# kevlar-dev/kevlar

Measured on AMD Instinct MI355X. Metric: reads/sec through count+novel (3 samples, k=31), higher is better.
Workload: dtype u64 hash / u8 counters

## Files before the change

### kevlar_amd/csrc/kv_skm.hip

```cpp
#include <algorithm>
#include <cmath>

#include "kv_binned.h"
#include "kv_novel_device.h"
#include "kv_skm_device.h"

struct SkmGeom {
    int k, m, w, wpow;
    int kw, nbw, recw, ncap;
    uint32_t C1, F2, fbits;
    uint32_t nwg1, nwg2, quota1;
    uint32_t cap1, cap2;
    uint32_t np_max;
    uint64_t stride;
    uint64_t *seg1; uint32_t *cnt1;
    uint64_t *seg2; uint32_t *cnt2;
    uint64_t *loose; uint64_t loose_cap;
    unsigned long long *ctr;
    uint32_t n_buckets, quota3;
    uint32_t sbw;
    uint64_t bucket_kmers;
    uint32_t force_loose;
    uint64_t *abl_keys; uint8_t *abl_cnts; uint32_t *abl_bstart, *abl_bcount; uint32_t abl_cap_wg;
    uint64_t *dl_keys, *dl_hash; uint32_t *dl_bstart, *dl_bcount; uint32_t dl_cap_wg;
// ... 1310 lines not shown
        while (longer) {
            const uint32_t src = (uint32_t)__ffsll((long long)longer) - 1u;
            longer &= longer - 1ull;
            const uint64_t b0 = skm_shfl64(bw[0], src), b1 = skm_shfl64(bw[1], src), b2 = skm_shfl64(bw[2], src);
            const uint32_t nk_src = (uint32_t)__shfl((int)nk, (int)src);
            for (uint32_t j0 = 0; j0 < nk_src; j0 += 64) {
                const uint32_t j = j0 + lane;
                const bool live = j < nk_src;
                count_one(skm_kmer_at<KW>(b0, b1, b2, live ? j : 0u, k), live);
            }
        }
    }
    n_added = wave_sum_u64(n_added);
    if ((threadIdx.x & 63) == 0 && n_added) atomicAdd(&g.ctr[BIN_CTR_ADDED], (unsigned long long)n_added);
}

#define SKM_ROUTE_MAX_DEST 16
struct SkmOverflowSink { unsigned long long *ctr; uint64_t *ovf; uint8_t *ovf_dest; uint64_t ovf_cap; int ndest; };
__device__ __attribute__((noinline)) void skm_route_overflow(SkmOverflowSink rs, uint32_t d, uint64_t h, uint64_t count)
{
    {
        const unsigned long long here = __ballot(true);
        const uint32_t lane = threadIdx.x & 63u, leader = (uint32_t)__ffsll((long long)here) - 1u;
        unsigned long long o = 0;
        if (lane == leader) o = atomicAdd(&rs.ctr[ROUTE_CTR_OVERFLOW], (unsigned long long)__popcll(here));
        o = skm_shfl64(o, leader) + (unsigned long long)__popcll(here & ((1ull << lane) - 1ull));
        const bool fits = o < rs.ovf_cap;
        for (int dd = 0; dd < rs.ndest; ++dd) {
            const unsigned long long same = __ballot(fits && d == (uint32_t)dd);
            if (same && lane == (uint32_t)__ffsll((long long)same) - 1u) atomicAdd(&rs.ctr[ROUTE_CTR_DEST0 + dd], (unsigned long long)__popcll(same));
        }
        if (fits) {
            *(ulonglong2 *)(rs.ovf + 2 * o) = make_ulonglong2(h, count);
            rs.ovf_dest[o] = (uint8_t)d;
        }
    }
}

__device__ __forceinline__ void skm_route_item(const KvRouteSink &rs, const uint64_t *lo, uint32_t *cur, uint64_t h, uint64_t count)
{
    if (h == UINT64_MAX) return;
    uint32_t d = 0;
    for (int b = 1; b < rs.ndest; ++b) d += h >= lo[b] ? 1u : 0u;
    const uint32_t pos = cur ? atomicAdd(&cur[d], 1u) : 0xffffffffu;
    if (pos < rs.seg_cap) *(ulonglong2 *)(rs.seg + (((uint64_t)d * rs.nwg + blockIdx.x) * rs.seg_cap + pos) * 2) = make_ulonglong2(h, count);
    else skm_route_overflow(SkmOverflowSink{rs.ctr, rs.ovf, rs.ovf_dest, rs.ovf_cap, rs.ndest}, d, h, count);
}

template <int KW, int TS, bool COMPACT = false>
__global__ __launch_bounds__(SKM_THREADS3, 6) void k_skm_route(SkmGeom sg, HashParams hp, KvRouteSink rs)
{
    __shared__ SkmTable<KW, TS> tb;
    __shared__ uint32_t cnt[TS];
    __shared__ uint32_t next_bucket;
    __shared__ uint32_t cur[SKM_ROUTE_MAX_DEST];
    __shared__ uint64_t lo[SKM_ROUTE_MAX_DEST];
    __shared__ uint32_t dl_cur, dl_b0, dl_prev;
    __shared__ uint32_t dl_org, dl_lim;
    extern __shared__ __attribute__((aligned(16))) uint32_t dyn[];
    uint32_t *lut = dyn, *scratch = dyn + 256;
    if (threadIdx.x < 256) lut[threadIdx.x] = skm_ascii4(threadIdx.x);
    if (threadIdx.x < (uint32_t)rs.ndest) { cur[threadIdx.x] = 0; lo[threadIdx.x] = rs.bs * (uint64_t)threadIdx.x; }
    const int k = sg.k;
    uint64_t n_distinct = 0;
    skm_table_clear(tb);
    for (uint32_t i = threadIdx.x; i < TS; i += SKM_THREADS3) cnt[i] = 0;
    if (threadIdx.x == 0) {
        next_bucket = (uint32_t)atomicAdd(&sg.ctr[SKM_CTR_TICKET_COUNT], 1ull) * sg.bpt; dl_cur = 0; dl_b0 = 0; dl_prev = 0xffffffffu;
        dl_org = sg.dl_chunk ? 0u : blockIdx.x * sg.dl_cap_wg; dl_lim = sg.dl_chunk ? 0u : sg.dl_cap_wg;
    }
    auto dl_close = [&]() {
        if (sg.dl_keys && dl_prev != 0xffffffffu) {
            sg.dl_bstart[dl_prev] = dl_org + dl_b0;
            sg.dl_bcount[dl_prev] = dl_cur - dl_b0;
            if (sg.dl_chunk && dl_cur > dl_lim) atomicAdd(&sg.ctr[SKM_CTR_DL_RAN_OUT], 1ull);
        }
    };
    auto passes_of = [&](uint32_t b) {
        const uint32_t least = sg.passes > 1u ? sg.passes : 1u;
        const uint32_t *cnt2 = sg.cnt2 + (uint64_t)b * sg.nwg2;
        uint32_t nrec = 0;
        for (uint32_t s2 = 0; s2 < sg.nwg2; ++s2) nrec += cnt2[s2];
        const uint32_t per_pass = (uint32_t)TS * 13u / 20u;
        const uint32_t want = (19u * nrec / 10u + per_pass - 1u) / per_pass;
        return min(64u, max(least, want));
    };
    for (uint32_t taken = 0; taken < sg.quota3; ++taken) {
        __syncthreads();
        const uint32_t b = next_bucket;
        if (b >= sg.n_buckets) break;
        __syncthreads();
        if (threadIdx.x == 0) {
            dl_close();
            if (sg.dl_keys && sg.dl_chunk) {
                const uint32_t need = passes_of(b) * (uint32_t)TS;
                if (dl_cur + need > dl_lim) {
                    const unsigned long long c = atomicAdd(&sg.ctr[SKM_CTR_POOL_CHUNKS], 1ull);
                    if (c < sg.dl_nchunks && need <= sg.dl_chunk) { dl_org = (uint32_t)c * sg.dl_chunk; dl_lim = sg.dl_chunk; }
                    else { dl_org = 0; dl_lim = 0; atomicAdd(&sg.ctr[SKM_CTR_DL_RAN_OUT], 1ull); }
                    dl_cur = 0;
                }
            }
            dl_prev = b; dl_b0 = dl_cur;
            if ((b + 1u) & (sg.bpt - 1u)) next_bucket = b + 1u;
            else if (taken + 1 >= sg.quota3 || __hip_atomic_load(&sg.ctr[SKM_CTR_FAIL], __ATOMIC_RELAXED, __HIP_MEMORY_SCOPE_AGENT) != 0) next_bucket = 0xffffffffu;
            else next_bucket = (uint32_t)atomicAdd(&sg.ctr[SKM_CTR_TICKET_COUNT], 1ull) * sg.bpt;
        }
        const uint32_t passes = passes_of(b);
        for (uint32_t pass = 0; pass < passes; ++pass) {
        if (pass) __syncthreads();
        skm_walk_bucket<KW, false, 0, COMPACT>(sg, b, scratch, [&](const SkmKey<KW> &c, uint64_t) {
            if (!skm_cacheable<KW>(c)) return pass == 0u;
            if (passes > 1u && __umulhi(skm_slot_hash<KW>(c) * 0x9E3779B1u, passes) != pass) return false;
            const int slot = skm_table_insert(tb, c);
            if (slot >= 0) atomicAdd(&cnt[slot], 1u);
            return slot < 0;
        });
        __syncthreads();
        skm_for_occupied<TS>(tb.key[0], (uint16_t *)scratch, skm_wave_scratch_words(sg.sbw) * 2u, [&](uint32_t slot) {
            SkmKey<KW> c;
            c.w[0] = tb.key[0][slot];
            tb.key[0][slot] = SKM_EMPTY;
            if (KW == 2) { c.w[KW - 1] = tb.key[KW - 1][slot]; tb.key[KW - 1][slot] = SKM_EMPTY; }
            const uint32_t seen = cnt[slot];
            cnt[slot] = 0;
            n_distinct += 1;
            const uint64_t h = skm_key_hash<KW>(c, lut, hp);
            if (sg.dl_keys) {
                const unsigned long long here = __ballot(true);
                const uint32_t lane = threadIdx.x & 63u, leader = (uint32_t)__ffsll((long long)here) - 1u;
                uint32_t base = 0;
                if (lane == leader) base = atomicAdd(&dl_cur, (uint32_t)__popcll(here));
                base = (uint32_t)__shfl((int)base, (int)leader);
                const uint32_t at = base + (uint32_t)__popcll(here & ((1ull << lane) - 1ull));
                if (at < dl_lim) {
                    const uint64_t e = (uint64_t)dl_org + at;
                    sg.dl_keys[e * KW] = c.w[0];
                    if (KW == 2) sg.dl_keys[e * KW + (KW - 1)] = c.w[KW - 1];
                    sg.dl_hash[e] = h;
                }
            }
            skm_route_item(rs, lo, cur, h, seen);
        });
        }
    }
    __syncthreads();
    if (threadIdx.x == 0) {
        dl_close();
        if (sg.dl_keys && !sg.dl_chunk && dl_cur > sg.dl_cap_wg) atomicAdd(&sg.ctr[SKM_CTR_DL_RAN_OUT], 1ull);
    }
    if (threadIdx.x < (uint32_t)rs.ndest)
        rs.seg_count[(uint64_t)threadIdx.x * rs.nwg + blockIdx.x] = (uint32_t)min((uint64_t)cur[threadIdx.x], rs.seg_cap);
    n_distinct = wave_sum_u64(n_distinct);
    if ((threadIdx.x & 63) == 0 && n_distinct) atomicAdd(&sg.ctr[SKM_CTR_DISTINCT], (unsigned long long)n_distinct);
}

template <int KW>
__global__ __launch_bounds__(256) void k_skm_loose_route(SkmGeom sg, HashParams hp, KvRouteSink rs)
{
    __shared__ uint32_t lut[256];
    __shared__ uint64_t lo[SKM_ROUTE_MAX_DEST];
    __shared__ uint32_t dcount[SKM_ROUTE_MAX_DEST];
    __shared__ uint32_t wg_items, wg_cur;
    __shared__ unsigned long long wg_base;
    if (sg.ctr[SKM_CTR_FAIL] != 0) return;
    lut[threadIdx.x] = skm_ascii4(threadIdx.x);
    if (threadIdx.x < SKM_ROUTE_MAX_DEST) { lo[threadIdx.x] = rs.bs * (uint64_t)threadIdx.x; dcount[threadIdx.x] = 0; }
    if (threadIdx.x == 0) { wg_items = 0; wg_cur = 0; }
    __syncthreads();
    unsigned long long n = sg.ctr[SKM_CTR_LOOSE];
    if (n > sg.loose_cap) n = sg.loose_cap;
    const int k = sg.k, recw = sg.lrecw;
    {
        uint32_t mine = 0;
        for (uint64_t i = blockIdx.x * (uint64_t)blockDim.x + threadIdx.x; i < n; i += (uint64_t)gridDim.x * blockDim.x)
            mine += skm_hdr_n(sg.loose[i * (uint64_t)recw]);
        if (mine) atomicAdd(&wg_items, mine);
    }
    __syncthreads();
    if (threadIdx.x == 0) wg_base = wg_items ? atomicAdd(&rs.ctr[ROUTE_CTR_OVERFLOW], (unsigned long long)wg_items) : 0ull;
    __syncthreads();
    for (uint64_t i = blockIdx.x * (uint64_t)blockDim.x + threadIdx.x; i < n; i += (uint64_t)gridDim.x * blockDim.x) {
        const uint64_t *rec = sg.loose + i * (uint64_t)recw;
        uint64_t bw[3];
#pragma unroll
        for (int t = 0; t < 3; ++t) bw[t] = t < sg.nbw ? rec[1 + t] : 0ull;
        const uint32_t nk = skm_hdr_n(rec[0]);
        SkmKey<KW> fw = skm_first_kmer<KW>(bw, k);
        SkmKey<KW> rc = skm_revcomp<KW>(fw, k);
        for (uint32_t j = 0; j < nk; ++j) {
            if (j) skm_roll<KW>(fw, rc, skm_base_at(bw, j + (uint32_t)k - 1u), k);
            const uint64_t h = skm_key_hash<KW>(skm_canonical<KW>(fw, rc), lut, hp);
            const unsigned long long o = wg_base + atomicAdd(&wg_cur, 1u);
            if (o >= rs.ovf_cap) continue;
            uint32_t d = 0;
            for (int b = 1; b < rs.ndest; ++b) d += h >= lo[b] ? 1u : 0u;
            if (h == UINT64_MAX) d = 0xffu;
            else atomicAdd(&dcount[d], 1u);
            *(ulonglong2 *)(rs.ovf + 2 * o) = make_ulonglong2(h, 1ull);
            rs.ovf_dest[o] = (uint8_t)d;
        }
    }
    __syncthreads();
    if (threadIdx.x < (uint32_t)rs.ndest && dcount[threadIdx.x]) atomicAdd(&rs.ctr[ROUTE_CTR_DEST0 + threadIdx.x], (unsigned long long)dcount[threadIdx.x]);
}

__device__ __forceinline__ void skm_mark(const NovelParams &p, const ReadsDev &rd, uint64_t pos, uint64_t stride)
{
    const uint64_t read = pos / stride;
    const uint64_t off = pos - read * stride;
    if ((rd.flags[read] & 1) || read < p.first_read) return;
    const uint64_t bit = read * p.mask_stride + off;
    atomicOr(&p.mask[bit >> 5], 1u << (bit & 31));
}

template <int KW, int TS>
__global__ __launch_bounds__(SKM_THREADS3, 6) void k_skm_novel(SkmGeom sg, ReadsDev rd, NovelParams p, SkmAblSet abls)
{
    __shared__ SkmTable<KW, TS> tb;
    __shared__ uint32_t flag[TS / 32];
    __shared__ uint32_t rej[TS / 32];
    __shared__ NovelShared ns;
    __shared__ uint32_t next_bucket, any_hit;
    extern __shared__ __attribute__((aligned(16))) uint32_t dyn[];
    uint32_t *lut = dyn, *scratch = dyn + 256;
    if (threadIdx.x < 256) lut[threadIdx.x] = skm_ascii4(threadIdx.x);
    load_descs(ns, p);
    const int k = sg.k;
    if (threadIdx.x == 0) next_bucket = (uint32_t)atomicAdd(&sg.ctr[SKM_CTR_TICKET_SCAN], 1ull) * sg.bpt;
    for (uint32_t taken = 0; taken < sg.quota3; ++taken) {
        __syncthreads();
        const uint32_t b = next_bucket;
        if (b >= sg.n_buckets) break;
        skm_table_clear(tb);
        if (threadIdx.x < TS / 32) { flag[threadIdx.x] = 0; rej[threadIdx.x] = 0; }
        __syncthreads();
        if (threadIdx.x == 0) {
            if ((b + 1u) & (sg.bpt - 1u)) next_bucket = b + 1u;
            else if (taken + 1 >= sg.quota3 || __hip_atomic_load(&sg.ctr[SKM_CTR_FAIL], __ATOMIC_RELAXED, __HIP_MEMORY_SCOPE_AGENT) != 0) next_bucket = 0xffffffffu;
            else {
                const unsigned long long ticket = atomicAdd(&sg.ctr[SKM_CTR_TICKET_SCAN], 1ull);
                next_bucket = (uint32_t)ticket * sg.bpt;
                const unsigned long long done = ticket * sg.bpt;
                if (done * 50ull >= sg.n_buckets) {
                    const unsigned long long now = __hip_atomic_load(&sg.ctr[SKM_CTR_LOOSE], __ATOMIC_RELAXED, __HIP_MEMORY_SCOPE_AGENT), start = sg.ctr[SKM_CTR_LOOSE_S12];
                    if (now > start && (now - start) * 25ull > done * sg.bucket_kmers) sg.ctr[SKM_CTR_FAIL] = 1;
                }
            }
            any_hit = 0;
        }
        skm_walk_bucket<KW, true, 0, false>(sg, b, scratch, [&](const SkmKey<KW> &c, uint64_t) {
            const int slot = skm_cacheable<KW>(c) ? skm_table_insert(tb, c) : -1;
            return slot < 0;
        });
        for (int a = 0; a < abls.n; ++a) {
            const uint32_t e0 = abls.bstart[a][b], en = abls.bcount[a][b];
            for (uint32_t i = threadIdx.x; i < en; i += SKM_THREADS3) {
                if ((int)min((uint32_t)abls.cnts[a][e0 + i], abls.maxv[a]) <= abls.ctrl_max) continue;
                SkmKey<KW> c;
                c.w[0] = abls.keys[a][(uint64_t)(e0 + i) * KW];
                if (KW == 2) c.w[KW - 1] = abls.keys[a][(uint64_t)(e0 + i) * KW + (KW - 1)];
                const int slot = skm_table_insert(tb, c);
                if (slot >= 0) atomicOr(&rej[slot >> 5], 1u << (slot & 31));
            }
        }
        __syncthreads();
        skm_for_occupied<TS>(tb.key[0], (uint16_t *)scratch, skm_wave_scratch_words(sg.sbw) * 2u, [&](uint32_t slot) {
            SkmKey<KW> c;
            c.w[0] = tb.key[0][slot];
            if (KW == 2) c.w[KW - 1] = tb.key[KW - 1][slot];
            const uint64_t h = skm_key_hash<KW>(c, lut, p.hp);
            if (band_pass(p, h) && novel_test_fast(ns, p, h, nullptr, 0ull)) { atomicOr(&flag[slot >> 5], 1u << (slot & 31)); any_hit = 1; }
        }, rej);
        __syncthreads();
        if (any_hit == 0) continue;
        skm_walk_bucket<KW, true, 0, false>(sg, b, scratch, [&](const SkmKey<KW> &c, uint64_t pos) {
            if (!skm_cacheable<KW>(c)) return false;
            const int slot = skm_table_find(tb, c);
            if (slot >= 0 && ((flag[slot >> 5] >> (slot & 31)) & 1u)) skm_mark(p, rd, pos, sg.stride);
            return false;
        });
    }
}

__global__ __launch_bounds__(256) void k_case_bits(const uint8_t *__restrict__ tab, uint64_t size, int case_min, uint32_t *__restrict__ bits)
{
    const uint64_t n_words = (size + 31) >> 5;
    for (uint64_t w = blockIdx.x * 256ull + threadIdx.x; w < n_words; w += (uint64_t)gridDim.x * 256ull) {
        uint32_t out = 0;
        if (w * 32 + 32 <= size) {
            const uint4 a = ((const uint4 *)tab)[2 * w], b = ((const uint4 *)tab)[2 * w + 1];
            const uint32_t q[8] = {a.x, a.y, a.z, a.w, b.x, b.y, b.z, b.w};
#pragma unroll
            for (int i = 0; i < 8; ++i)
#pragma unroll
                for (int j = 0; j < 4; ++j) out |= ((int)((q[i] >> (8 * j)) & 0xffu) >= case_min ? 1u : 0u) << (4 * i + j);
        } else {
            for (uint64_t j = w * 32; j < size; ++j) out |= ((int)tab[j] >= case_min ? 1u : 0u) << (uint32_t)(j - w * 32);
        }
        bits[w] = out;
    }
}

template <int KW, int TSM>
__global__ __launch_bounds__(SKM_THREADS3, 6) void k_skm_novel_list(SkmGeom sg, ReadsDev rd, NovelParams p, SkmAblSet abls)
{
    constexpr uint32_t E = 4;
    __shared__ SkmTable<KW, TSM> rtb;
    __shared__ SkmTable<KW, TSM> itb;
    __shared__ NovelShared ns;
    __shared__ uint16_t cand[SKM_LIST_MAX];
    __shared__ uint32_t next_bucket, n_int, n_cand;
    extern __shared__ __attribute__((aligned(16))) uint32_t dyn[];
    uint32_t *scratch = dyn;
    load_descs(ns, p);
    skm_table_clear(itb);
    if (threadIdx.x == 0) { next_bucket = (uint32_t)atomicAdd(&sg.ctr[SKM_CTR_TICKET_SCAN], 1ull) * sg.bpt; n_int = 0; n_cand = 0; }
    auto mark_pass = [&](uint32_t b) {
        skm_walk_bucket<KW, true, 0, false>(sg, b, scratch, [&](const SkmKey<KW> &c, uint64_t pos) {
            if (skm_cacheable<KW>(c) && skm_table_find(itb, c) >= 0) skm_mark(p, rd, pos, sg.stride);
            return false;
        });
        __syncthreads();
        skm_table_clear(itb);
        if (threadIdx.x == 0) n_int = 0;
        __syncthreads();
    };
    for (uint32_t taken = 0; taken < sg.quota3; ++taken) {
        __syncthreads();
        const uint32_t b = next_bucket;
        if (b >= sg.n_buckets) break;
        skm_table_clear(rtb);
        __syncthreads();
        if (threadIdx.x == 0) {
            if ((b + 1u) & (sg.bpt - 1u)) next_bucket = b + 1u;
            else if (taken + 1 >= sg.quota3 || __hip_atomic_load(&sg.ctr[SKM_CTR_FAIL], __ATOMIC_RELAXED, __HIP_MEMORY_SCOPE_AGENT) != 0) next_bucket = 0xffffffffu;
            else next_bucket = (uint32_t)atomicAdd(&sg.ctr[SKM_CTR_TICKET_SCAN], 1ull) * sg.bpt;
            n_cand = 0;
        }
        const uint32_t e0 = sg.dl_bstart[b], en = min(sg.dl_bcount[b], SKM_LIST_MAX);
        SkmKey<KW> c[E];
        uint64_t h[E];
        auto request = [&](uint32_t base) {
#pragma unroll
            for (uint32_t u = 0; u < E; ++u) {
                const uint32_t i = base + u * SKM_THREADS3 + threadIdx.x;
                const bool in = i < en;
                c[u].w[0] = in ? sg.dl_keys[(uint64_t)(e0 + i) * KW] : SKM_EMPTY;
                if (KW == 2) c[u].w[KW - 1] = in ? sg.dl_keys[(uint64_t)(e0 + i) * KW + (KW - 1)] : SKM_EMPTY;
                h[u] = in ? sg.dl_hash[e0 + i] : 0ull;
            }
        };
        request(0);
        for (int a = 0; a < abls.n; ++a) {
            const uint32_t a0 = abls.bstart[a][b], an = abls.bcount[a][b];
            for (uint32_t i = threadIdx.x; i < an; i += SKM_THREADS3) {
                if ((int)min((uint32_t)abls.cnts[a][a0 + i], abls.maxv[a]) <= abls.ctrl_max) continue;
                SkmKey<KW> c;
                c.w[0] = abls.keys[a][(uint64_t)(a0 + i) * KW];
                if (KW == 2) c.w[KW - 1] = abls.keys[a][(uint64_t)(a0 + i) * KW + (KW - 1)];
                (void)skm_table_insert(rtb, c);
            }
        }
        __syncthreads();
        for (uint32_t e0 = 0; e0 < en; e0 += E * SKM_THREADS3) {
            if (e0) request(e0);
            bool live[E];
            uint32_t v[E];
#pragma unroll
            for (uint32_t u = 0; u < E; ++u) {
                live[u] = e0 + u * SKM_THREADS3 + threadIdx.x < en && skm_table_find(rtb, c[u]) < 0 && band_pass(p, h[u]);
                if (p.case0_bits) {
                    const uint64_t bin = fastmod(h[u], ns.d[0].size, ns.d[0].magic);
                    const __attribute__((address_space(1))) uint32_t *bits = (const __attribute__((address_space(1))) uint32_t *)p.case0_bits;
                    v[u] = live[u] && ((bits[bin >> 5] >> (uint32_t)(bin & 31u)) & 1u) ? (uint32_t)p.case_min : 0u;
                } else {
                    v[u] = live[u] ? probe(ns, 0, 0, h[u]) : 0u;
                }
            }
#pragma unroll
            for (uint32_t u = 0; u < E; ++u)
                if (live[u] && (int)v[u] >= p.case_min) cand[atomicAdd(&n_cand, 1u)] = (uint16_t)(e0 + u * SKM_THREADS3 + threadIdx.x);
        }
        __syncthreads();
        const uint32_t nc = n_cand;
        for (uint32_t j0 = 0; j0 < nc; j0 += SKM_THREADS3) {
            const uint32_t j = j0 + threadIdx.x;
            if (j < nc) {
                const uint32_t i = cand[j];
                SkmKey<KW> c;
                c.w[0] = sg.dl_keys[(uint64_t)(e0 + i) * KW];
                if (KW == 2) c.w[KW - 1] = sg.dl_keys[(uint64_t)(e0 + i) * KW + (KW - 1)];
                const uint64_t h = sg.dl_hash[e0 + i];
                if (novel_test_wide(ns, p, h)) {
                    if (skm_table_insert(itb, c) < 0) sg.ctr[SKM_CTR_FAIL] = 1;
                    atomicAdd(&n_int, 1u);
                    if (p.ab_keys) (void)ab_claim(p, h, p.ncase + p.nctrl);
                }
            }
            __syncthreads();
            if (n_int > TSM / 4 && j0 + SKM_THREADS3 < nc) mark_pass(b);
        }
        if (n_int != 0) mark_pass(b);
    }
}

__global__ __launch_bounds__(256) void k_ab_fill(NovelParams p)
{
    __shared__ NovelShared ns;
    load_descs(ns, p);
    __syncthreads();
    const int S = p.ncase + p.nctrl;
    const unsigned int listed = p.ab_list ? *p.ab_count : 0xffffffffu;
    if (listed <= p.ab_list_cap) {
        for (uint64_t i = blockIdx.x * 256ull + threadIdx.x; i < listed; i += (uint64_t)gridDim.x * 256ull) {
            const uint64_t slot = p.ab_list[i];
            hit_abundances(ns, p, (uint64_t)p.ab_keys[slot], p.ab_vals + slot * (uint64_t)S);
        }
        return;
    }
    for (uint64_t slot = blockIdx.x * 256ull + threadIdx.x; slot <= p.ab_mask; slot += (uint64_t)gridDim.x * 256ull) {
        const unsigned long long h = p.ab_keys[slot];
        if (h != 0ull) hit_abundances(ns, p, (uint64_t)h, p.ab_vals + slot * (uint64_t)S);
    }
}

template <int KW>
__global__ __launch_bounds__(256) void k_skm_loose_novel(SkmGeom sg, ReadsDev rd, NovelParams p)
{
    __shared__ uint32_t lut[256];
    __shared__ NovelShared ns;
    lut[threadIdx.x] = skm_ascii4(threadIdx.x);
    load_descs(ns, p);
    __syncthreads();
    unsigned long long n = sg.ctr[SKM_CTR_LOOSE];
    if (n > sg.loose_cap) n = sg.loose_cap;
    const int k = sg.k, recw = sg.lrecw;
    const uint32_t lane = threadIdx.x & 63u;
    auto test_one = [&](const SkmKey<KW> &fw, bool live, uint64_t pos) {
        if (!live) return;
        const uint64_t h = skm_key_hash<KW>(skm_canonical<KW>(fw, skm_revcomp<KW>(fw, k)), lut, p.hp);
        if (band_pass(p, h) && novel_test_fast(ns, p, h, nullptr, 0ull)) skm_mark(p, rd, pos, sg.stride);
    };
    const uint64_t total_waves = (uint64_t)gridDim.x * (blockDim.x >> 6), wave_id = (uint64_t)blockIdx.x * (blockDim.x >> 6) + (threadIdx.x >> 6);
    const uint32_t per = (uint32_t)min((unsigned long long)64, max((unsigned long long)1, (n + total_waves - 1) / total_waves));
    for (uint64_t i0 = wave_id * per; i0 < n; i0 += total_waves * per) {
        const uint64_t i = i0 + lane;
        const bool have = lane < per && i < n;
        const uint64_t *rec = sg.loose + (have ? i : 0) * (uint64_t)recw;
        uint64_t bw[3];
#pragma unroll
        for (int t = 0; t < 3; ++t) bw[t] = (have && t < sg.nbw) ? rec[1 + t] : 0ull;
        const uint64_t hdr = have ? rec[0] : 0ull;
        const uint32_t nk = have ? skm_hdr_n(hdr) : 0u;
        test_one(skm_first_kmer<KW>(bw, k), nk == 1, skm_hdr_pos_of(hdr, 0u));
        unsigned long long longer = __ballot(nk > 1);
        while (longer) {
            const uint32_t src = (uint32_t)__ffsll((long long)longer) - 1u;
            longer &= longer - 1ull;
            const uint64_t b0 = skm_shfl64(bw[0], src), b1 = skm_shfl64(bw[1], src), b2 = skm_shfl64(bw[2], src), h_src = skm_shfl64(hdr, src);
            const uint32_t nk_src = (uint32_t)__shfl((int)nk, (int)src);
            for (uint32_t j0 = 0; j0 < nk_src; j0 += 64) {
                const uint32_t j = j0 + lane;
                const bool live = j < nk_src;
                test_one(skm_kmer_at<KW>(b0, b1, b2, live ? j : 0u, k), live, skm_hdr_pos_of(h_src, live ? j : 0u));
            }
        }
    }
}

struct SetHitSink {
    unsigned long long *tags;
    uint8_t *abund;
    unsigned long long *count;
    uint64_t cap;
};
__device__ __forceinline__ void set_hit_store(const NovelParams &p, const SetHitSink &out, uint64_t at, unsigned long long tag, uint64_t slot)
{
    if (at >= out.cap) return;
    const int S = p.ncase + p.nctrl;
    out.tags[at] = tag;
    for (int c = 0; c < S; ++c) out.abund[at * (uint64_t)S + c] = p.set_abund[slot * (uint64_t)S + c];
}
#define SKM_HIT_STAGE 1024u
template <int KW, int TSM>
__global__ __launch_bounds__(SKM_THREADS3, 6) void k_skm_set_hits(SkmGeom sg, NovelParams p, SetHitSink out)
{
    __shared__ SkmTable<KW, TSM> itb;
    __shared__ uint32_t islot[TSM];
    __shared__ unsigned long long htag[SKM_HIT_STAGE];
    __shared__ uint32_t hslot[SKM_HIT_STAGE];
    __shared__ uint32_t next_bucket, n_int, n_hit;
    __shared__ unsigned long long flush_base;
    extern __shared__ __attribute__((aligned(16))) uint32_t dyn[];
    uint32_t *scratch = dyn;
    skm_table_clear(itb);
    if (threadIdx.x == 0) { next_bucket = (uint32_t)atomicAdd(&sg.ctr[SKM_CTR_TICKET_SCAN], 1ull) * sg.bpt; n_int = 0; n_hit = 0; }
    for (uint32_t taken = 0; taken < sg.quota3; ++taken) {
        __syncthreads();
        const uint32_t b = next_bucket;
        if (b >= sg.n_buckets) break;
        __syncthreads();
        if (threadIdx.x == 0) {
            if ((b + 1u) & (sg.bpt - 1u)) next_bucket = b + 1u;
            else if (taken + 1 >= sg.quota3) next_bucket = 0xffffffffu;
            else next_bucket = (uint32_t)atomicAdd(&sg.ctr[SKM_CTR_TICKET_SCAN], 1ull) * sg.bpt;
        }
        const uint32_t e0 = sg.dl_bstart[b], en = sg.dl_bcount[b];
        for (uint32_t i = threadIdx.x; i < en; i += SKM_THREADS3) {
            const uint64_t h = sg.dl_hash[e0 + i];
            const uint64_t slot = set_find(p, h);
            if (slot == KV_SET_NONE) continue;
            SkmKey<KW> c;
            c.w[0] = sg.dl_keys[(uint64_t)(e0 + i) * KW];
            if (KW == 2) c.w[KW - 1] = sg.dl_keys[(uint64_t)(e0 + i) * KW + (KW - 1)];
            const int at = skm_table_insert(itb, c);
            if (at < 0) { sg.ctr[SKM_CTR_FAIL] = 1; continue; }
            islot[at] = (uint32_t)slot;
            atomicAdd(&n_int, 1u);
        }
        __syncthreads();
        if (n_int == 0) continue;
        skm_walk_bucket<KW, true, 0, false>(sg, b, scratch, [&](const SkmKey<KW> &c, uint64_t pos) {
            if (!skm_cacheable<KW>(c)) return false;
            const int at = skm_table_find(itb, c);
            if (at < 0) return false;
            const uint64_t read = pos / sg.stride;
            const unsigned long long tag = ((unsigned long long)read << 16) | (unsigned long long)(pos - read * sg.stride);
            const uint32_t i = atomicAdd(&n_hit, 1u);
            if (i < SKM_HIT_STAGE) { htag[i] = tag; hslot[i] = islot[at]; }
            else set_hit_store(p, out, atomicAdd(out.count, 1ull), tag, islot[at]);
            return false;
        });
        __syncthreads();
        const uint32_t staged = min(n_hit, SKM_HIT_STAGE);
        if (threadIdx.x == 0) flush_base = atomicAdd(out.count, (unsigned long long)staged);
        skm_table_clear(itb);
        __syncthreads();
        for (uint32_t i = threadIdx.x; i < staged; i += SKM_THREADS3) set_hit_store(p, out, flush_base + i, htag[i], hslot[i]);
        if (threadIdx.x == 0) { n_int = 0; n_hit = 0; }
    }
}

template <int KW>
__global__ __launch_bounds__(256) void k_skm_loose_set_hits(SkmGeom sg, NovelParams p, SetHitSink out)
{
    __shared__ uint32_t lut[256];
    lut[threadIdx.x] = skm_ascii4(threadIdx.x);
    __syncthreads();
    unsigned long long n = sg.ctr[SKM_CTR_LOOSE];
    if (n > sg.loose_cap) n = sg.loose_cap;
    const int k = sg.k, recw = sg.lrecw;
    for (uint64_t i = blockIdx.x * (uint64_t)blockDim.x + threadIdx.x; i < n; i += (uint64_t)gridDim.x * blockDim.x) {
        const uint64_t *rec = sg.loose + i * (uint64_t)recw;
        uint64_t bw[3];
#pragma unroll
        for (int t = 0; t < 3; ++t) bw[t] = t < sg.nbw ? rec[1 + t] : 0ull;
        const uint32_t nk = skm_hdr_n(rec[0]);
        SkmKey<KW> fw = skm_first_kmer<KW>(bw, k);
        SkmKey<KW> rc = skm_revcomp<KW>(fw, k);
        for (uint32_t j = 0; j < nk; ++j) {
            if (j) skm_roll<KW>(fw, rc, skm_base_at(bw, j + (uint32_t)k - 1u), k);
            const uint64_t slot = set_find(p, skm_key_hash<KW>(skm_canonical<KW>(fw, rc), lut, p.hp));
            if (slot == KV_SET_NONE) continue;
            const uint64_t pos = skm_hdr_pos_of(rec[0], j), read = pos / sg.stride;
            set_hit_store(p, out, atomicAdd(out.count, 1ull), ((unsigned long long)read << 16) | (unsigned long long)(pos - read * sg.stride), slot);
        }
    }
}

__global__ void k_skm_forward_flag(const unsigned long long *skm_ctr, unsigned long long *bin_ctr)
{
    if (skm_ctr[SKM_CTR_FAIL] != 0) bin_ctr[BIN_CTR_FAIL] = 1;
}

__global__ __launch_bounds__(64) void k_tile_hits(ReadsDev rd, NovelParams p)
{
    const TileDesc td = rd.tile[blockIdx.x];
    uint64_t b0, b1;
    if (td.seg) {
        b0 = (uint64_t)td.first * p.mask_stride + td.seg_start;
        b1 = min(b0 + (uint64_t)KV_SEG_BASES, ((uint64_t)td.first + 1) * p.mask_stride);
    } else {
        b0 = (uint64_t)td.first * p.mask_stride;
        b1 = ((uint64_t)td.first + td.count) * p.mask_stride;
    }
    uint64_t n = 0;
    for (uint64_t w = (b0 >> 5) + threadIdx.x; w < ((b1 + 31) >> 5); w += 64) {
        uint32_t bits = p.mask[w];
        const uint64_t wlo = w << 5;
        if (wlo < b0) bits &= ~0u << (uint32_t)(b0 - wlo);
        if (wlo + 32 > b1) bits &= b1 > wlo ? (~0u >> (uint32_t)(wlo + 32 - b1)) : 0u;
        n += (uint32_t)__popc(bits);
    }
    n = wave_sum_u64(n);
    if (threadIdx.x == 0) p.tile_count[blockIdx.x] = (uint32_t)n;
}

struct SkmCarve {
    unsigned char *base;
    size_t total = 0;
    explicit SkmCarve(void *arena = nullptr) : base((unsigned char *)arena) {}
    template <typename T> T *take(size_t bytes) { T *p = (T *)base; bytes = kv_round_up(bytes, 256); total += bytes; if (base) base += bytes; return p; }
};

template <typename V> size_t skm_list_lay(SkmCarve c, uint64_t entries, int kw, uint32_t n_buckets, uint64_t **keys, V **vals, uint32_t **bstart, uint32_t **bcount)
{
    *keys = c.take<uint64_t>(entries * 8 * kw); *vals = c.take<V>(entries * sizeof(V));
    *bstart = c.take<uint32_t>((uint64_t)n_buckets * 4); *bcount = c.take<uint32_t>((uint64_t)n_buckets * 4);
    return c.total;
}
hipError_t skm_list_zero(uint32_t *bstart, uint32_t *bcount, hipStream_t st) { return hipMemsetAsync(bstart, 0, (size_t)((unsigned char *)bcount - (unsigned char *)bstart) * 2, st); }

struct SkmDistinctList {
    uint64_t *keys = nullptr, *hash = nullptr;
    uint32_t *bstart = nullptr, *bcount = nullptr;
    uint32_t cap_wg = 0, chunk = 0, nchunks = 0;
    static size_t bytes(uint64_t entries, int kw, uint32_t n_buckets) { SkmDistinctList l; return skm_list_lay(SkmCarve(), entries, kw, n_buckets, &l.keys, &l.hash, &l.bstart, &l.bcount); }
    int carve(KvArena &arena, uint64_t entries, int kw, uint32_t n_buckets, uint32_t cap_wg_, uint32_t chunk_, uint32_t nchunks_, hipStream_t st)
    {
        if (arena.need(bytes(entries, kw, n_buckets)) != hipSuccess) return KV_ERR_CAPACITY;
        skm_list_lay(SkmCarve(arena.p), entries, kw, n_buckets, &keys, &hash, &bstart, &bcount);
        cap_wg = cap_wg_; chunk = chunk_; nchunks = nchunks_;
        KV_HIP(skm_list_zero(bstart, bcount, st));
        return KV_OK;
    }
    void attach(SkmGeom &g) const { g.dl_keys = keys; g.dl_hash = hash; g.dl_bstart = bstart; g.dl_bcount = bcount; g.dl_cap_wg = cap_wg; g.dl_chunk = chunk; g.dl_nchunks = nchunks; }
    static void detach(SkmGeom &g) { g.dl_keys = nullptr; g.dl_hash = nullptr; g.dl_bstart = nullptr; g.dl_bcount = nullptr; }
};
void skm_abl_attach(const KvAbundList &al, SkmGeom &g) { g.abl_keys = al.keys; g.abl_cnts = al.cnts; g.abl_bstart = al.bstart; g.abl_bcount = al.bcount; g.abl_cap_wg = (uint32_t)al.cap_wg; }
void skm_abl_detach(SkmGeom &g) { g.abl_keys = nullptr; g.abl_cnts = nullptr; g.abl_bstart = nullptr; g.abl_bcount = nullptr; }

struct SkmIndex {
    KvArena arena;
    uint64_t reads_uid = 0;
    int k = 0;
    bool valid = false;
    double distinct_hint = 0.0;
    SkmGeom g;
    KvArena dl;
    size_t dl_refused = SIZE_MAX;
    SkmDistinctList list;
    bool dl_valid = false;
    bool mex_scan_ready = false;
    uint64_t builds = 0;
    KvArena bits;
    std::mutex mu;
    enum { BATCH = 1, MEX_SCAN = 2, LIST = 4, ALL = 7 };
    void drop(int what) { valid &= !(what & BATCH); mex_scan_ready &= !(what & MEX_SCAN); dl_valid &= !(what & LIST); }
    void give_back() { drop(ALL); arena.release(); dl.release(); list = SkmDistinctList(); }
};
std::map<hipStream_t, SkmIndex> g_skm;
std::mutex g_skm_mu;
int g_skm_pref_k = 0;
uint64_t g_skm_pref_nfine = 0;
double g_skm_last_distinct = 0.0;

SkmIndex &skm_index_for(hipStream_t st)
{
    std::lock_guard<std::mutex> lk(g_skm_mu);
    return g_skm[kv_stream_key(st)];
}
}
void kv_skm_scratch_release()
{
    std::lock_guard<std::mutex> lk(g_skm_mu);
    for (auto &kv : g_skm) {
        SkmIndex &idx = kv.second;
        std::lock_guard<std::mutex> ilk(idx.mu);
        idx.give_back();
        idx.bits.release();
    }
}
namespace {

inline uint32_t skm_nwg3(const SkmGeom &g)
{
    return (uint32_t)std::min<uint64_t>((g.n_buckets + g.bpt - 1) / g.bpt, 3u * (uint32_t)kv_device_cus());
}

static void skm_plan_tickets(SkmGeom &g)
{
    g.bpt = SKM_BUCKETS_PER_TICKET;
    while (g.bpt > 2u && g.n_buckets / g.bpt < 4u * 768u) g.bpt /= 2u;
    const uint32_t nwg3 = skm_nwg3(g);
    const uint64_t avg = (g.n_buckets + nwg3 - 1) / nwg3;
    g.quota3 = (uint32_t)kv_round_up(avg + avg / 2 + 1, g.bpt);
}

inline uint32_t pow2_ceil(uint64_t v) { uint32_t p = 1; while (p < v) p <<= 1; return p; }

static void skm_bucket_grid(uint64_t nfine, uint32_t *C1, uint32_t *F2, uint32_t *fbits)
{
    *F2 = std::min<uint32_t>(512u, pow2_ceil((uint64_t)std::ceil(std::sqrt((double)nfine))));
    if (nfine > 255ull * *F2) *F2 = std::min<uint32_t>(SKM_MAX_F2, pow2_ceil((nfine + 254) / 255));
    *fbits = 0;
    while ((1u << *fbits) < *F2) ++*fbits;
    *C1 = (uint32_t)std::min<uint64_t>(255, std::max<uint64_t>(1, (nfine + *F2 - 1) / *F2));
}

static double skm_rec_est(uint64_t n_kmers, double n_reads, int w) { return (double)n_kmers * 2.2 / (double)(w + 1) + n_reads + 1024.0; }
static uint32_t skm_seg_cap(double mean, double slack, uint64_t floor) { return (uint32_t)kv_round_up((uint64_t)(mean * slack + 8.0 * std::sqrt(mean)) + floor, 16); }
static uint64_t skm_loose_cap(double rec_est, uint64_t n_kmers) { return (uint64_t)(rec_est / 8.0) + n_kmers / 16 + (1u << 20); }
static uint32_t skm_sbw(int ncap) { return ((64u * (uint32_t)ncap) >> 5) + 2u; }
static void skm_make_compact(SkmGeom &g) { g.compact = 1u; g.recw = 2; g.ncap = std::min(g.ncap, SKM_C_BASES + 1 - g.k); g.sbw = skm_sbw(g.ncap); }

// ... 894 lines not shown
```

Before: 1.015 billion.

## Prefetch next bucket descriptors and cache candidate keys in shared memory

Double-buffers per-bucket descriptors (list start/count and each ABL's start/count) in shared memory, fetching the next bucket's values with the first wavefront while the current bucket is processed. This takes the dependent global loads off the critical path at each bucket start. Candidate keys and hashes are also stashed in a small shared side buffer so the novel-test phase skips re-reading them from global memory. The rtb clear moves after the scan, and one barrier in mark_pass is dropped on the final pass. The cost is extra shared memory, which can lower occupancy, plus a more complex synchronisation order.

```diff
diff --git a/kevlar_amd/csrc/kv_skm.hip b/kevlar_amd/csrc/kv_skm.hip
--- a/kevlar_amd/csrc/kv_skm.hip
+++ b/kevlar_amd/csrc/kv_skm.hip
@@ -1636,21 +1636,43 @@
     }
 }
 
+#define SKM_LS_DESC (3 + 2 * SKM_MAX_ABL)
 template <int KW, int TSM>
 __global__ __launch_bounds__(SKM_THREADS3, 6) void k_skm_novel_list(SkmGeom sg, ReadsDev rd, NovelParams p, SkmAblSet abls)
 {
     constexpr uint32_t E = 4;
+    constexpr uint32_t SIDE = 128 / KW;
     __shared__ SkmTable<KW, TSM> rtb;
     __shared__ SkmTable<KW, TSM> itb;
     __shared__ NovelShared ns;
     __shared__ uint16_t cand[SKM_LIST_MAX];
-    __shared__ uint32_t next_bucket, n_int, n_cand;
+    __shared__ unsigned long long side_key[KW][SIDE], side_hash[SIDE];
+    __shared__ uint32_t desc[2][SKM_LS_DESC];
+    __shared__ uint32_t n_int, n_cand;
     extern __shared__ __attribute__((aligned(16))) uint32_t dyn[];
     uint32_t *scratch = dyn;
     load_descs(ns, p);
     skm_table_clear(itb);
-    if (threadIdx.x == 0) { next_bucket = (uint32_t)atomicAdd(&sg.ctr[SKM_CTR_TICKET_SCAN], 1ull) * sg.bpt; n_int = 0; n_cand = 0; }
-    auto mark_pass = [&](uint32_t b) {
+    skm_table_clear(rtb);
+    auto desc_fetch = [&](uint32_t nb) {
+        const uint32_t *src = nullptr;
+        if (threadIdx.x == 1) src = sg.dl_bstart;
+        if (threadIdx.x == 2) src = sg.dl_bcount;
+#pragma unroll
+        for (int a = 0; a < SKM_MAX_ABL; ++a) {
+            if (a < abls.n && threadIdx.x == 3u + 2u * a) src = abls.bstart[a];
+            if (a < abls.n && threadIdx.x == 4u + 2u * a) src = abls.bcount[a];
+        }
+        return nb < sg.n_buckets && src ? src[nb] : nb;
+    };
+    if (threadIdx.x < 64) {
+        uint32_t nb = 0;
+        if (threadIdx.x == 0) { nb = (uint32_t)atomicAdd(&sg.ctr[SKM_CTR_TICKET_SCAN], 1ull) * sg.bpt; n_int = 0; n_cand = 0; }
+        nb = (uint32_t)__shfl((int)nb, 0);
+        const uint32_t v = desc_fetch(nb);
+        if (threadIdx.x < SKM_LS_DESC) desc[0][threadIdx.x] = v;
+    }
+    auto mark_pass = [&](uint32_t b, bool more) {
         skm_walk_bucket<KW, true, 0, false>(sg, b, scratch, [&](const SkmKey<KW> &c, uint64_t pos) {
             if (skm_cacheable<KW>(c) && skm_table_find(itb, c) >= 0) skm_mark(p, rd, pos, sg.stride);
             return false;
@@ -1658,21 +1680,26 @@
         __syncthreads();
         skm_table_clear(itb);
         if (threadIdx.x == 0) n_int = 0;
-        __syncthreads();
+        if (more) __syncthreads();
     };
     for (uint32_t taken = 0; taken < sg.quota3; ++taken) {
         __syncthreads();
-        const uint32_t b = next_bucket;
+        const uint32_t *dq = desc[taken & 1u];
+        const uint32_t b = dq[0];
         if (b >= sg.n_buckets) break;
-        skm_table_clear(rtb);
-        __syncthreads();
-        if (threadIdx.x == 0) {
-            if ((b + 1u) & (sg.bpt - 1u)) next_bucket = b + 1u;
-            else if (taken + 1 >= sg.quota3 || __hip_atomic_load(&sg.ctr[SKM_CTR_FAIL], __ATOMIC_RELAXED, __HIP_MEMORY_SCOPE_AGENT) != 0) next_bucket = 0xffffffffu;
-            else next_bucket = (uint32_t)atomicAdd(&sg.ctr[SKM_CTR_TICKET_SCAN], 1ull) * sg.bpt;
-            n_cand = 0;
-        }
-        const uint32_t e0 = sg.dl_bstart[b], en = min(sg.dl_bcount[b], SKM_LIST_MAX);
+        const uint32_t e0 = dq[1], en = min(dq[2], SKM_LIST_MAX);
+        uint32_t dnext = 0;
+        if (threadIdx.x < 64) {
+            uint32_t nb = 0;
+            if (threadIdx.x == 0) {
+                if ((b + 1u) & (sg.bpt - 1u)) nb = b + 1u;
+                else if (taken + 1 >= sg.quota3 || __hip_atomic_load(&sg.ctr[SKM_CTR_FAIL], __ATOMIC_RELAXED, __HIP_MEMORY_SCOPE_AGENT) != 0) nb = 0xffffffffu;
+                else nb = (uint32_t)atomicAdd(&sg.ctr[SKM_CTR_TICKET_SCAN], 1ull) * sg.bpt;
+                n_cand = 0;
+            }
+            nb = (uint32_t)__shfl((int)nb, 0);
+            dnext = desc_fetch(nb);
+        }
         SkmKey<KW> c[E];
         uint64_t h[E];
         auto request = [&](uint32_t base) {
@@ -1687,13 +1714,13 @@
         };
         request(0);
         for (int a = 0; a < abls.n; ++a) {
-            const uint32_t a0 = abls.bstart[a][b], an = abls.bcount[a][b];
+            const uint32_t a0 = dq[3 + 2 * a], an = dq[4 + 2 * a];
             for (uint32_t i = threadIdx.x; i < an; i += SKM_THREADS3) {
-                if ((int)min((uint32_t)abls.cnts[a][a0 + i], abls.maxv[a]) <= abls.ctrl_max) continue;
+                const bool over = (int)min((uint32_t)abls.cnts[a][a0 + i], abls.maxv[a]) > abls.ctrl_max;
                 SkmKey<KW> c;
                 c.w[0] = abls.keys[a][(uint64_t)(a0 + i) * KW];
                 if (KW == 2) c.w[KW - 1] = abls.keys[a][(uint64_t)(a0 + i) * KW + (KW - 1)];
-                (void)skm_table_insert(rtb, c);
+                if (over & (c.w[0] != SKM_EMPTY)) (void)skm_table_insert(rtb, c);
             }
         }
         __syncthreads();
@@ -1714,18 +1741,36 @@
             }
 #pragma unroll
             for (uint32_t u = 0; u < E; ++u)
-                if (live[u] && (int)v[u] >= p.case_min) cand[atomicAdd(&n_cand, 1u)] = (uint16_t)(e0 + u * SKM_THREADS3 + threadIdx.x);
-        }
-        __syncthreads();
+                if (live[u] && (int)v[u] >= p.case_min) {
+                    const uint32_t at = atomicAdd(&n_cand, 1u);
+                    cand[at] = (uint16_t)(e0 + u * SKM_THREADS3 + threadIdx.x);
+                    if (at < SIDE) {
+                        side_key[0][at] = c[u].w[0];
+                        if (KW == 2) side_key[KW - 1][at] = c[u].w[KW - 1];
+                        side_hash[at] = h[u];
+                    }
+                }
+        }
+        if (threadIdx.x < SKM_LS_DESC) desc[(taken & 1u) ^ 1u][threadIdx.x] = dnext;
+        __syncthreads();
+        skm_table_clear(rtb);
         const uint32_t nc = n_cand;
         for (uint32_t j0 = 0; j0 < nc; j0 += SKM_THREADS3) {
+            const bool last_round = j0 + SKM_THREADS3 >= nc;
             const uint32_t j = j0 + threadIdx.x;
             if (j < nc) {
-                const uint32_t i = cand[j];
                 SkmKey<KW> c;
-                c.w[0] = sg.dl_keys[(uint64_t)(e0 + i) * KW];
-                if (KW == 2) c.w[KW - 1] = sg.dl_keys[(uint64_t)(e0 + i) * KW + (KW - 1)];
-                const uint64_t h = sg.dl_hash[e0 + i];
+                uint64_t h;
+                if (j < SIDE) {
+                    c.w[0] = side_key[0][j];
+                    if (KW == 2) c.w[KW - 1] = side_key[KW - 1][j];
+                    h = side_hash[j];
+                } else {
+                    const uint32_t i = cand[j];
+                    c.w[0] = sg.dl_keys[(uint64_t)(e0 + i) * KW];
+                    if (KW == 2) c.w[KW - 1] = sg.dl_keys[(uint64_t)(e0 + i) * KW + (KW - 1)];
+                    h = sg.dl_hash[e0 + i];
+                }
                 if (novel_test_wide(ns, p, h)) {
                     if (skm_table_insert(itb, c) < 0) sg.ctr[SKM_CTR_FAIL] = 1;
                     atomicAdd(&n_int, 1u);
@@ -1733,9 +1778,9 @@
                 }
             }
             __syncthreads();
-            if (n_int > TSM / 4 && j0 + SKM_THREADS3 < nc) mark_pass(b);
-        }
-        if (n_int != 0) mark_pass(b);
+            if (n_int > TSM / 4 && !last_round) mark_pass(b, true);
+        }
+        if (n_int != 0) mark_pass(b, false);
     }
 }
 
```

Result: no change. 1.022 billion (median of 6 runs) (+0.7%).
